# raufs/skDER

Hardware: NVIDIA B200
Metric: genome pairs/sec ANI+AF (higher is better)
Workload: dtype u64/int32 + f64

## Files before the change

### skder_b200/build.py

```python
import os
import subprocess
import sys

HERE = os.path.dirname(os.path.abspath(__file__))
CSRC = os.path.join(HERE, "csrc")
LIBDIR = os.path.join(HERE, "_lib")
LIB = os.path.join(LIBDIR, "libskani_b200.so")
SOURCES = ["skb_api.cu", "fasta_pack.cpp"]
HEADERS = ["skb_common.cuh", "skb_sketch.cuh", "skb_index.cuh", "skb_probe.cuh", "skb_ani.cuh", "../../include/skani_b200.h"]


def _stale():
    if not os.path.exists(LIB):
        return True
    t = os.path.getmtime(LIB)
    return any(os.path.getmtime(os.path.join(CSRC, f)) > t for f in SOURCES + HEADERS)


def build(force=False, verbose=False):
    if not force and not _stale():
        return LIB
    os.makedirs(LIBDIR, exist_ok=True)
    nvcc = os.environ.get("NVCC", "/usr/local/cuda/bin/nvcc")
    cmd = [
        nvcc, "-O3", "-std=c++17",
        "-gencode", "arch=compute_100a,code=sm_100a",
        "-lineinfo", "-Xcompiler", "-fPIC", "-shared",
        "-o", LIB,
    ] + [os.path.join(CSRC, s) for s in SOURCES] + ["-lz"]
    if verbose:
        cmd.insert(1, "-Xptxas=-v")
        print(" ".join(cmd), file=sys.stderr)
    subprocess.check_call(cmd)
    return LIB


if __name__ == "__main__":
    print(build(force="--force" in sys.argv, verbose=True))
```

### skder_b200/csrc/skb_api.cu

```cuda
#include <cuda_runtime.h>

#include <algorithm>
#include <cmath>
#include <cstdio>
#include <cstdlib>
#include <cstring>
#include <ctime>
#include <cub/cub.cuh>
#include <map>
#include <string>
#include <thread>
#include <vector>

#include "skb_ani.cuh"
#include "skb_common.cuh"
#include "skb_index.cuh"
#include "skb_sketch.cuh"

using namespace skb;

namespace {

thread_local std::string g_create_error;

struct CudaFail {
    std::string msg;
};

#define CK(call)                                                                                          \
    do {                                                                                                  \
        cudaError_t e__ = (call);                                                                         \
        if (e__ != cudaSuccess)                                                                           \
            throw CudaFail{std::string(#call) + ": " + cudaGetErrorString(e__) + " (" + __FILE__ + ":" + \
                           std::to_string(__LINE__) + ")"};                                               \
    } while (0)

template <typename T>
struct DevBuf {
    T *p = nullptr;
    size_t cap = 0;
    ~DevBuf() { release(); }
    void release() {
        if (p) cudaFree(p);
        p = nullptr;
        cap = 0;
    }
    void reserve(size_t n, size_t keep, cudaStream_t st) {
        if (n <= cap) return;
        size_t ncap = std::max(n, cap + cap / 2);
        T *q = nullptr;
        CK(cudaMalloc(&q, ncap * sizeof(T)));
        if (p && keep) CK(cudaMemcpyAsync(q, p, keep * sizeof(T), cudaMemcpyDeviceToDevice, st));
        if (p) {
            CK(cudaStreamSynchronize(st));
            cudaFree(p);
        }
        p = q;
        cap = ncap;
    }
    void upload(const std::vector<T> &h, size_t from, cudaStream_t st) {
        reserve(std::max<size_t>(h.size(), 1), from, st);
        if (h.size() > from)
            CK(cudaMemcpyAsync(p + from, h.data() + from, (h.size() - from) * sizeof(T), cudaMemcpyHostToDevice, st));
    }
};

template <typename T>
struct PoolRef {
    DevBuf<unsigned char> &b;
// ... 41 lines not shown
        int32_t n() const { return (int32_t)total_len.size(); }
        template <typename L>
        void append(uint64_t n_seeds, uint64_t len, const L *ctg_lens, size_t n_ctg) {
            seed_off.push_back(seed_off.back() + n_seeds);
            total_len.push_back(len);
            for (size_t k = 0; k < n_ctg; k++) ctg_len.push_back((uint32_t)ctg_lens[k]);
            ctg_off.push_back((uint32_t)ctg_len.size());
        }
        void truncate(int32_t n, uint64_t mkeys) {
            seed_off.resize(n + 1);
            total_len.resize(n);
            ctg_off.resize(n + 1);
            ctg_len.resize(ctg_off.back());
            n_mkeys = mkeys;
        }
        void clear() { *this = SketchDb(); }
    } db;
    struct HostIndex {
        int32_t n_indexed = 0;
        int32_t n_inv_genomes = 0;
        uint64_t n_inv = 0;
        uint64_t n_mkeys_indexed = 0;
        std::vector<uint64_t> tab_off{0}, marker_off{0};
        std::vector<uint32_t> chunk_off{0};
        std::vector<uint32_t> tab_buckets;
        std::vector<uint32_t> ctg_pstart, chunk_start, chunk_len;

        void truncate(const SketchDb &db) {
            const int32_t n = db.n();
            if (n_indexed <= n) return;
            n_indexed = n;
            tab_off.resize(n + 1);
            tab_buckets.resize(n);
            ctg_pstart.resize(db.ctg_len.size());
            chunk_off.resize(n + 1);
            chunk_start.resize(chunk_off.back());
            chunk_len.resize(chunk_off.back());
            marker_off.resize(n + 1);
            n_mkeys_indexed = std::min(n_mkeys_indexed, db.n_mkeys);
        }
        void clear() { *this = HostIndex(); }
    } ix;
    DevBuf<uint64_t> d_seeds, d_mkeys;
    bool indexed = false;
    int32_t own_first = 0, own_count = -1;
    int32_t kept_n = 0;
    uint64_t kept_seeds = 0;
    int kept_x2 = 0;
    int tab_x2 = 4;
    int tab_x2_forced = 0;
    int x2_decided = 0;
    uint64_t x2_decided_seeds = 0;
    DevBuf<uint64_t> d_seed_off, d_tab, d_tab_off, d_total_len, d_inv, d_markers, d_marker_off;
    DevBuf<uint32_t> d_tab_buckets;
    DevBuf<uint32_t> d_chunk_begin, d_chunk_start, d_chunk_len, d_chunk_off, d_ctg_pstart, d_ctg_len, d_ctg_off,
        d_marker_cnt;
    struct AddCall { int32_t n_before; uint64_t mkeys_before; };
    std::vector<AddCall> add_calls;
    DevBuf<unsigned char> d_tmp;
    std::map<std::string, DevBuf<unsigned char>> pool;
    DevBuf<int> d_counter;
    DevBuf<PairInfo> d_info;
    DevBuf<uint32_t> d_nch, d_task_off;

    int32_t n() const { return db.n(); }
    bool owns(int32_t g) const { return own_count < 0 || (g >= own_first && g < own_first + own_count); }
    std::pair<int32_t, int32_t> owned_in(int32_t g0, int32_t n) const {
        const int32_t o0 = std::clamp(own_count < 0 ? g0 : own_first, g0, n);
        return {o0, std::clamp(own_count < 0 ? n : own_first + own_count, o0, n)};
    }
    DbView view() const {
        DbView v;
        v.n_genomes = ix.n_indexed;
        v.seeds = d_seeds.p;
        v.g_seed_off = d_seed_off.p;
        v.tab = d_tab.p;
        v.g_tab_off = d_tab_off.p;
        v.g_tab_buckets = d_tab_buckets.p;
        v.chunk_begin = d_chunk_begin.p;
        v.chunk_start = d_chunk_start.p;
        v.chunk_len = d_chunk_len.p;
        v.g_chunk_off = d_chunk_off.p;
        v.ctg_pstart = d_ctg_pstart.p;
        v.ctg_len = d_ctg_len.p;
        v.g_ctg_off = d_ctg_off.p;
        v.g_total_len = d_total_len.p;
        v.markers = d_markers.p;
        v.g_marker_off = d_marker_off.p;
        v.inv_keys = d_inv.p;
        v.n_inv = (int64_t)ix.n_inv;
        return v;
    }
    AniParams ani_params() const {
        AniParams a;
        a.band_bp = prm.band_bp;
        a.max_gap = prm.max_gap;
        a.anchor_score = prm.anchor_score;
        a.min_anchors = prm.min_anchors;
        a.min_score = prm.min_score;
        a.max_mult = prm.max_mult;
        a.max_chunk_chains = prm.max_chunk_chains;
        a.ovl_num = prm.ovl_num;
        a.ovl_den = prm.ovl_den;
        a.span_ext = prm.span_ext;
        a.debias_a = prm.debias_a;
        a.debias_g = prm.debias_g;
        return a;
    }
};

namespace {

template <typename F>
int guarded(skb_ctx *ctx, F &&f) {
    if (!ctx) return SKB_EINVAL;
    try {
        CK(cudaSetDevice(ctx->device));
        return f();
    } catch (const CudaFail &e) {
        ctx->err = e.msg;
        return SKB_ECUDA;
    } catch (const std::bad_alloc &) {
        ctx->err = "host out of memory";
        return SKB_ENOMEM;
    } catch (const std::exception &e) {
        ctx->err = e.what();
        return SKB_EINVAL;
    }
// ... 100 lines not shown
    CK(cudaGetLastError());
    c->launches++;
    exclusive_scan_u32(c, d_cnt_s.p, d_off_s.p, n_warps + 1);
    exclusive_scan_u32(c, d_cnt_m.p, d_off_m.p, n_warps + 1);
    std::vector<uint32_t> h_off_s(nb + 1);
    uint32_t tot_m = 0;
    PoolRef<uint32_t> d_goff(c->pool["sketch_batch.d_goff"]);
    d_goff.reserve((size_t)nb + 1, 0, c->st);
    gather_strided_kernel<<<nblk((uint64_t)nb + 1, 256), 256, 0, c->st>>>(d_off_s.p, b.tile_off, SK_WARPS, nb + 1, d_goff.p);
    CK(cudaGetLastError());
    c->launches++;
    CK(cudaMemcpyAsync(h_off_s.data(), d_goff.p, ((size_t)nb + 1) * 4, cudaMemcpyDeviceToHost, c->st));
    CK(cudaMemcpyAsync(&tot_m, d_off_m.p + n_warps, 4, cudaMemcpyDeviceToHost, c->st));
    CK(cudaStreamSynchronize(c->st));
    const uint64_t cur_seeds = c->db.seed_off.back();
    const uint64_t tot_s = h_off_s[nb];
    c->d_seeds.reserve(cur_seeds + tot_s + 1, cur_seeds, c->st);
    c->d_mkeys.reserve(c->db.n_mkeys + tot_m + 1, c->db.n_mkeys, c->st);
    sketch_kernel<true><<<n_tiles, SK_THREADS, 0, c->st>>>(b, nullptr, nullptr, d_off_s.p, d_off_m.p,
                                                           c->d_seeds.p + cur_seeds, c->d_mkeys.p + c->db.n_mkeys,
                                                           d_masks.p);
    CK(cudaGetLastError());
    c->launches++;
    CK(cudaStreamSynchronize(c->st));
    for (int32_t i = 0; i < nb; i++) {
        const skb_packed *p = gen[g0 + i];
        c->db.append(h_off_s[i + 1] - h_off_s[i], (uint64_t)p->n_bases, p->contig_lens, (size_t)p->n_contigs);
    }
    c->db.n_mkeys += tot_m;
    c->indexed = false;
}

constexpr int EST_SORT_LAUNCHES = 4;

void run_ani(skb_ctx *c, const unsigned long long *d_pairs, int64_t n_pairs, PairOut *d_out) {
    c->anchor_ev_used = 0;
    if (n_pairs == 0) return;
    if (n_pairs >= (1ll << 31)) throw CudaFail{"too many surviving pairs in one call"};
    static const uint32_t fw_cap = [] {
        const char *e = std::getenv("SKB_FW_CAP");
        const int v = e ? atoi(e) : 1024;
        uint32_t w = 32;
        while ((int)w < v && w < 4096) w <<= 1;
        return w;
    }();
    const size_t fw_smem = (size_t)FW_WARPS * ((fw_bytes_per_warp(fw_cap) + 15) & ~(size_t)15);
    if (!c->ani_attr_set) {
        CK(cudaFuncSetAttribute(finalize_kernel<false, false>, cudaFuncAttributeMaxDynamicSharedMemorySize,
                                (int)(FIN_BYTES_PER_CAND * MAXP)));
        CK(cudaFuncSetAttribute(finalize_kernel<false, true>, cudaFuncAttributeMaxDynamicSharedMemorySize,
                                (int)(FIN_BYTES_PER_CAND * MAXP)));
        CK(cudaFuncSetAttribute(finalize_warp_kernel<false>, cudaFuncAttributeMaxDynamicSharedMemorySize, (int)fw_smem));
        CK(cudaFuncSetAttribute(finalize_warp_kernel<true>, cudaFuncAttributeMaxDynamicSharedMemorySize, (int)fw_smem));
        c->ani_attr_set = true;
    }
    const bool est = c->estimator != SKB_ANI_MEAN;
    const DbView view = c->view();
    const AniParams prm = c->ani_params();
    c->d_info.reserve((size_t)n_pairs, 0, c->st);
    c->d_nch.reserve((size_t)n_pairs + 1, 0, c->st);
    c->d_task_off.reserve((size_t)n_pairs + 1, 0, c->st);
    PoolRef<unsigned long long> d_key(c->pool["run_ani.key"]), d_key2(c->pool["run_ani.key2"]);
    PoolRef<uint32_t> d_idx(c->pool["run_ani.idx"]), d_perm(c->pool["run_ani.perm"]);
    PoolRef<PairInfo> d_info_s(c->pool["run_ani.info_sorted"]);
    d_key.reserve((size_t)n_pairs, 0, c->st);
    d_key2.reserve((size_t)n_pairs, 0, c->st);
    d_idx.reserve((size_t)n_pairs, 0, c->st);
    d_perm.reserve((size_t)n_pairs, 0, c->st);
    d_info_s.reserve((size_t)n_pairs, 0, c->st);
    pair_setup_kernel<<<nblk((uint64_t)n_pairs, 256), 256, 0, c->st>>>(view, d_pairs, n_pairs, c->d_info.p, d_key.p,
                                                                      d_idx.p);
    CK(cudaGetLastError());
    {
        size_t bytes = 0;
        CK(cub::DeviceRadixSort::SortPairs(nullptr, bytes, d_key.p, d_key2.p, d_idx.p, d_perm.p, (int64_t)n_pairs, 0, 64,
                                           c->st));
        c->d_tmp.reserve(bytes + 16, 0, c->st);
        CK(cub::DeviceRadixSort::SortPairs(c->d_tmp.p, bytes, d_key.p, d_key2.p, d_idx.p, d_perm.p, (int64_t)n_pairs, 0,
                                           64, c->st));
    }
    pair_gather_kernel<<<nblk((uint64_t)n_pairs, 256), 256, 0, c->st>>>(c->d_info.p, d_perm.p, n_pairs, d_info_s.p,
                                                                       c->d_nch.p);
    CK(cudaGetLastError());
    c->launches += 11;
    CK(cudaMemsetAsync(c->d_nch.p + n_pairs, 0, 4, c->st));
    exclusive_scan_u32(c, c->d_nch.p, c->d_task_off.p, (size_t)n_pairs + 1);
    std::vector<uint32_t> h_nch((size_t)n_pairs);
    CK(cudaMemcpyAsync(h_nch.data(), c->d_nch.p, (size_t)n_pairs * 4, cudaMemcpyDeviceToHost, c->st));
    CK(cudaStreamSynchronize(c->st));
    uint64_t total_tasks = 0;
    for (uint32_t v : h_nch) total_tasks += v;
    static const uint64_t batch_tasks = [] {
        const char *e = std::getenv("SKB_PAIR_BATCH_TASKS");
        return (uint64_t)(e ? std::max(1 << 16, atoi(e)) : (5 << 20));
    }();
    const uint64_t want_batches = std::max<uint64_t>(1, (total_tasks + batch_tasks / 2) / batch_tasks);
    const uint64_t max_tasks = std::min<uint64_t>(8ull << 20, (total_tasks + want_batches - 1) / want_batches + 4096);
    struct Batch { int64_t p0, p1; uint64_t base, tasks; };
    std::vector<Batch> batches;
    {
        int64_t p0 = 0;
        uint64_t base = 0;
        while (p0 < n_pairs) {
            uint64_t tasks = 0;
            int64_t p1 = p0;
            while (p1 < n_pairs && (p1 == p0 || tasks + h_nch[(size_t)p1] <= max_tasks)) tasks += h_nch[(size_t)p1++];
            if (tasks >= (1ull << 32)) throw CudaFail{"one pair has more than 2^32 query chunks"};
            batches.push_back({p0, p1, base, tasks});
            base += tasks;
            p0 = p1;
        }
    }
    uint64_t cap = 1;
    int64_t cap_pairs = 1;
    for (const Batch &bt : batches) {
        cap = std::max(cap, bt.tasks);
        cap_pairs = std::max(cap_pairs, bt.p1 - bt.p0);
    }
    PoolRef<uint64_t> b_anc(c->pool["ani.anc"]);
    PoolRef<uint32_t> b_res(c->pool["ani.res"]), b_next(c->pool["ani.next"]), b_fctl(c->pool["ani.fin_ctl"]),
        b_big_list(c->pool["ani.big_list"]), b_big_nc(c->pool["ani.big_nc"]), b_mid_list(c->pool["ani.mid_list"]);
    PoolRef<uint16_t> b_tn(c->pool["ani.tn"]);
    PoolRef<TaskDesc> b_desc(c->pool["ani.desc"]);
    PoolRef<Cand> b_cands(c->pool["ani.cands"]);
    PoolRef<PCand> b_pcands(c->pool["ani.pcands"]);
    PoolRef<uint32_t> b_task_pair(c->pool["ani.task_pair"]), b_cand_off(c->pool["ani.cand_off"]);
    PoolRef<uint8_t> b_ncand(c->pool["ani.ncand"]);
    PoolRef<uint32_t> b_slow(c->pool["ani.slow_list"]);
    b_anc.reserve(slab_entries(cap) + 2, 0, c->st);
    b_res.reserve(slab_entries(cap), 0, c->st);
    b_tn.reserve((size_t)cap, 0, c->st);
    b_desc.reserve((size_t)cap, 0, c->st);
    b_cands.reserve((size_t)cap * SLOTS, 0, c->st);
    b_pcands.reserve((size_t)cap * SLOTS, 0, c->st);
    b_task_pair.reserve((size_t)cap, 0, c->st);
    b_cand_off.reserve((size_t)cap + 1, 0, c->st);
    b_ncand.reserve((size_t)cap + 1, 0, c->st);
    b_slow.reserve((size_t)cap + 1, 0, c->st);
    b_next.reserve(1, 0, c->st);
    b_fctl.reserve(4, 0, c->st);
    b_mid_list.reserve((size_t)cap_pairs, 0, c->st);
    b_big_list.reserve((size_t)cap_pairs, 0, c->st);
    b_big_nc.reserve((size_t)cap_pairs, 0, c->st);
    PoolRef<uint8_t> e_acc(c->pool["est.acc"]);
    if (est) e_acc.reserve((size_t)cap * SLOTS, 0, c->st);
    bool wide_diag = std::getenv("SKB_WIDE_DIAG") != nullptr && atoi(std::getenv("SKB_WIDE_DIAG")) != 0;
    for (int32_t g = 0; g < c->ix.n_indexed && !wide_diag; g++) {
        const uint32_t k1 = c->db.ctg_off[(size_t)g + 1];
        if (k1 > c->db.ctg_off[(size_t)g] &&
            (uint64_t)c->ix.ctg_pstart[k1 - 1] + c->db.ctg_len[k1 - 1] >= (1ull << 30) - (1ull << 21))
            wide_diag = true;
    }
    static const bool trace = std::getenv("SKB_TRACE") != nullptr;
    struct Span { const char *name; size_t batch; cudaEvent_t e0, e1; };
    std::vector<Span> spans;
    cudaEvent_t ev_t0 = nullptr;
    auto mark = [&]() {
        cudaEvent_t e = nullptr;
        if (trace) {
            CK(cudaEventCreate(&e));
            CK(cudaEventRecord(e, c->st));
        }
        return e;
    };
    if (trace) ev_t0 = mark();
    for (size_t bi = 0; bi < batches.size(); bi++) {
        const Batch &bt = batches[bi];
        const int64_t np = bt.p1 - bt.p0;
        const uint32_t tasks = (uint32_t)bt.tasks, base = (uint32_t)bt.base;
        CK(cudaMemsetAsync(b_fctl.p, 0, 16, c->st));
        if (tasks) {
            CK(cudaMemsetAsync(b_ncand.p, 0, (size_t)tasks + 1, c->st));
            CK(cudaMemsetAsync(b_slow.p, 0, 4, c->st));
            CK(cudaMemsetAsync(b_next.p, 0, 4, c->st));
            task_setup_kernel<<<nblk(tasks, 256), 256, 0, c->st>>>(view, d_info_s.p + bt.p0, c->d_task_off.p + bt.p0, base, np,
                                                                   tasks, b_desc.p, b_task_pair.p);
            CK(cudaGetLastError());
            const unsigned g1 = std::min<unsigned>(nblk(tasks, (ANC_THREADS / 32) * ANC_GRAB), (unsigned)c->sm_count * 32u);
            if ((int)c->anchor_ev.size() < c->anchor_ev_used + 2) {
                cudaEvent_t e0, e1;
                CK(cudaEventCreate(&e0));
                CK(cudaEventCreate(&e1));
                c->anchor_ev.push_back(e0);
                c->anchor_ev.push_back(e1);
            }
            CK(cudaEventRecord(c->anchor_ev[c->anchor_ev_used], c->st));
            cudaEvent_t t0 = mark();
            if (wide_diag)
                anchor_kernel<false><<<g1, ANC_THREADS, 0, c->st>>>(view, prm, b_desc.p, tasks, b_anc.p, b_tn.p, b_next.p);
            else
                anchor_kernel<true><<<g1, ANC_THREADS, 0, c->st>>>(view, prm, b_desc.p, tasks, b_anc.p, b_tn.p, b_next.p);
            CK(cudaGetLastError());
            if (trace) spans.push_back({"anchor", bi, t0, mark()});
            CK(cudaEventRecord(c->anchor_ev[c->anchor_ev_used + 1], c->st));
            c->anchor_ev_used += 2;
            t0 = mark();
            if (wide_diag)
                chain_kernel<true><<<nblk(tasks, DP_THREADS), DP_THREADS, 0, c->st>>>(prm, tasks, b_anc.p, b_tn.p, b_res.p, b_desc.p,
                                                                                      b_cands.p, b_ncand.p, b_slow.p);
            else
                chain_kernel<false><<<nblk(tasks, DP_THREADS), DP_THREADS, 0, c->st>>>(prm, tasks, b_anc.p, b_tn.p, b_res.p, b_desc.p,
                                                                                       b_cands.p, b_ncand.p, b_slow.p);
            CK(cudaGetLastError());
            if (trace) spans.push_back({"chain", bi, t0, mark()});
            const unsigned g3 = std::min<unsigned>(nblk(tasks, END_THREADS / 32), (unsigned)c->sm_count * 4u);
            ends_kernel<<<g3, END_THREADS, 0, c->st>>>(prm, tasks, b_anc.p, b_res.p, b_tn.p, b_desc.p, b_slow.p, b_cands.p,
                                                       b_ncand.p);
            CK(cudaGetLastError());
            c->launches += 4;
        }
        cudaEvent_t tf = mark();
        if (tasks) {
            exclusive_scan_u8(c, b_ncand.p, b_cand_off.p, (size_t)tasks + 1);
            cand_pack_kernel<<<nblk(tasks, 256), 256, 0, c->st>>>(view, prm, d_info_s.p + bt.p0, tasks, b_task_pair.p, b_ncand.p,
                                                                  b_cand_off.p, b_cands.p, b_pcands.p);
            CK(cudaGetLastError());
            c->launches += 1;
        }
        (est ? finalize_warp_kernel<true> : finalize_warp_kernel<false>)<<<nblk((uint64_t)np, FW_WARPS), FW_WARPS * 32, fw_smem,
                                                                          c->st>>>(
            view, prm, d_info_s.p + bt.p0, c->d_task_off.p + bt.p0, base, np, b_pcands.p, b_cand_off.p, d_perm.p + bt.p0, d_out,
            fw_cap, b_fctl.p, b_mid_list.p, b_big_list.p, b_big_nc.p, e_acc.p);
        CK(cudaGetLastError());
        uint32_t fctl[4] = {0, 0, 0, 0};
        uint32_t n_cand = 0;
        CK(cudaMemcpyAsync(fctl, b_fctl.p, 16, cudaMemcpyDeviceToHost, c->st));
        if (est && tasks) CK(cudaMemcpyAsync(&n_cand, b_cand_off.p + tasks, 4, cudaMemcpyDeviceToHost, c->st));
        CK(cudaStreamSynchronize(c->st));
        c->launches += 1;
        if (fctl[2]) {
            uint32_t fcap = 32;
            while (fcap < fctl[0]) fcap <<= 1;
            (est ? finalize_kernel<false, true> : finalize_kernel<false, false>)<<<fctl[2], FIN_THREADS,
                                                                                  FIN_BYTES_PER_CAND * (size_t)fcap, c->st>>>(
                view, prm, d_info_s.p + bt.p0, c->d_task_off.p + bt.p0, base, np, b_pcands.p, b_cand_off.p,
                d_perm.p + bt.p0, d_out, fcap, b_mid_list.p, nullptr, nullptr, nullptr, e_acc.p);
            CK(cudaGetLastError());
            c->launches += 1;
        }
        if (fctl[1]) {
            const uint32_t nbig = fctl[1];
// ... 375 lines not shown
}


static int table_density(skb_ctx *c, uint64_t own_seeds) {
    if (c->tab_x2_forced) return c->tab_x2_forced;
    if (c->x2_decided && c->x2_decided_seeds == own_seeds) return c->x2_decided;
    size_t free_b = 0, total_b = 0;
    CK(cudaMemGetInfo(&free_b, &total_b));
    const double budget = std::min(0.35 * (double)total_b,
                                   (double)free_b + (double)c->d_tab.cap * 8.0 - 40.0 * (double)(1ull << 30));
    c->x2_decided = 1;
    for (int x2 : {4, 2})
        if (((double)own_seeds * x2 / 2 + (double)c->n()) * BUCKET * 8.0 <= budget) {
            c->x2_decided = x2;
            break;
        }
    c->x2_decided_seeds = own_seeds;
    return c->x2_decided;
}

static int build_seed_tables(skb_ctx *c, int32_t g0, bool reuse) {
    const int32_t n = c->n();
    std::vector<uint64_t> &tab_off = c->ix.tab_off;
    std::vector<uint32_t> &buckets = c->ix.tab_buckets;
    tab_off.resize(n + 1);
    buckets.resize(n);
    for (int32_t g = g0; g < n; g++) {
        const uint64_t ns = c->db.seed_off[g + 1] - c->db.seed_off[g];
        if (ns >= (1ull << 31)) return fail(c, SKB_ELIMIT, "genome has too many seeds");
        buckets[g] = c->owns(g) ? (uint32_t)std::max<uint64_t>(2, ns * (uint64_t)c->tab_x2 / 2 + 1) : 0u;
        tab_off[g + 1] = tab_off[g] + (uint64_t)buckets[g] * BUCKET;
    }
    c->d_seed_off.upload(c->db.seed_off, g0, c->st);
    c->d_tab_off.upload(tab_off, g0, c->st);
    c->d_tab_buckets.upload(buckets, g0, c->st);
    const uint64_t t0 = tab_off[g0], t1 = tab_off[n];
    c->d_tab.reserve(t1 + BUCKET, reuse ? t1 : t0, c->st);
    if (reuse) return SKB_OK;
    CK(cudaMemsetAsync(c->d_tab.p + t0, 0xFF, (t1 - t0) * 8, c->st));
    const auto [o0, o1] = c->owned_in(g0, n);
    const uint64_t s0 = c->db.seed_off[o0], s1 = c->db.seed_off[o1];
    if (s1 > s0) {
        tab_insert_kernel<<<nblk(s1 - s0, 256), 256, 0, c->st>>>(c->d_seeds.p, s1, c->d_seed_off.p, n, c->d_tab.p,
                                                               c->d_tab_off.p, c->d_tab_buckets.p, s0);
        CK(cudaGetLastError());
        rep_flag_kernel<<<nblk(s1 - s0, 256), 256, 0, c->st>>>(c->d_seeds.p, s1, c->d_seed_off.p, n, c->d_tab.p,
                                                             c->d_tab_off.p, c->d_tab_buckets.p, c->prm.max_mult, s0);
        CK(cudaGetLastError());
        c->launches += 2;
    }
    return SKB_OK;
}

static int build_chunk_tables(skb_ctx *c, int32_t g0) {
    const int32_t n = c->n();
    const uint32_t CL = (uint32_t)c->prm.chunk_len;
    const skb_ctx::SketchDb &db = c->db;
    skb_ctx::HostIndex &ix = c->ix;
    ix.chunk_off.resize(n + 1);
    for (int32_t g = g0; g < n; g++) {
        uint64_t cnt = 0;
        for (uint32_t k = db.ctg_off[g]; k < db.ctg_off[g + 1]; k++) cnt += (db.ctg_len[k] + CL - 1) / CL;
        if ((uint64_t)ix.chunk_off[g] + cnt >= (1ull << 32)) return fail(c, SKB_ELIMIT, "too many chunks");
        ix.chunk_off[g + 1] = ix.chunk_off[g] + (uint32_t)cnt;
    }
    ix.ctg_pstart.resize(db.ctg_len.size());
    ix.chunk_start.resize(ix.chunk_off[n]);
    ix.chunk_len.resize(ix.chunk_off[n]);
    auto fill = [&](int32_t ga, int32_t gb) {
        for (int32_t g = ga; g < gb; g++) {
            uint32_t off = 0, at = ix.chunk_off[g];
            for (uint32_t k = db.ctg_off[g]; k < db.ctg_off[g + 1]; k++) {
                ix.ctg_pstart[k] = off;
                const uint32_t len = db.ctg_len[k];
                for (uint32_t st = 0; st < len; st += CL, at++) {
                    ix.chunk_start[at] = off + st;
                    ix.chunk_len[at] = std::min<uint32_t>(CL, len - st);
                }
                off += len + CONTIG_PAD;
            }
        }
    };
    const int64_t m = n - g0;
    const int n_thr = m >= 1024 ? 4 : 1;
    if (n_thr == 1)
        fill(g0, n);
    else {
        std::vector<std::thread> pool;
        for (int t = 0; t < n_thr; t++)
            pool.emplace_back(fill, g0 + (int32_t)(m * t / n_thr), g0 + (int32_t)(m * (t + 1) / n_thr));
        for (auto &th : pool) th.join();
    }
    const size_t k0 = db.ctg_off[g0], ch0 = ix.chunk_off[g0];
    c->d_total_len.upload(db.total_len, g0, c->st);
    c->d_ctg_off.upload(db.ctg_off, g0, c->st);
    c->d_ctg_len.upload(db.ctg_len, k0, c->st);
    c->d_ctg_pstart.upload(ix.ctg_pstart, k0, c->st);
    c->d_chunk_off.upload(ix.chunk_off, g0, c->st);
    c->d_chunk_start.upload(ix.chunk_start, ch0, c->st);
    c->d_chunk_len.upload(ix.chunk_len, ch0, c->st);
    const uint32_t e0 = (uint32_t)ch0 + (uint32_t)g0, e1 = ix.chunk_off[n] + (uint32_t)n;
    c->d_chunk_begin.reserve(e1, e0, c->st);
    chunk_begin_kernel<<<nblk(e1 - e0, 256), 256, 0, c->st>>>(c->d_seeds.p, c->d_seed_off.p, c->d_chunk_off.p, n,
                                                             c->d_chunk_start.p, c->d_chunk_begin.p, e1, e0);
    CK(cudaGetLastError());
    c->launches++;
    return SKB_OK;
}

static void marker_offsets(skb_ctx *c, int32_t g0) {
    const int32_t n = c->n();
    std::vector<uint32_t> cnt((size_t)(n - g0));
    CK(cudaMemcpyAsync(cnt.data(), c->d_marker_cnt.p + g0, cnt.size() * 4, cudaMemcpyDeviceToHost, c->st));
    CK(cudaStreamSynchronize(c->st));
    std::vector<uint64_t> &off = c->ix.marker_off;
    off.resize(n + 1);
    for (int32_t g = g0; g < n; g++) off[g + 1] = off[g] + cnt[(size_t)(g - g0)];
    c->d_marker_off.upload(off, g0, c->st);
    CK(cudaStreamSynchronize(c->st));
}

int skb_index(skb_ctx *ctx) {
    return guarded(ctx, [&]() -> int {
        skb_ctx *c = ctx;
        static const bool trace = std::getenv("SKB_TRACE") != nullptr;
        double t_last = 0;
        auto lap = [&](const char *what) {
            if (!trace) return;
            cudaStreamSynchronize(c->st);
            timespec ts;
            clock_gettime(CLOCK_MONOTONIC, &ts);
            const double now = ts.tv_sec * 1e3 + ts.tv_nsec * 1e-6;
            if (what) fprintf(stderr, "[skb trace] index %-14s %7.2f ms\n", what, now - t_last);
            t_last = now;
        };
        lap(nullptr);
        const int32_t n = c->n();
        if (n == 0) return fail(c, SKB_ESTATE, "no genomes added");
        const auto [o0, o1] = c->owned_in(0, n);
        const uint64_t own_seeds = c->db.seed_off[o1] - c->db.seed_off[o0];
        const bool reuse = c->kept_n > 0 && c->kept_n == o1 - o0 && c->kept_seeds == own_seeds;
        c->tab_x2 = reuse ? c->kept_x2 : table_density(c, own_seeds);
        int rc = build_seed_tables(c, 0, reuse);
        if (rc != SKB_OK) return rc;
        c->kept_n = 0;
        lap("seed tables");
        if ((rc = build_chunk_tables(c, 0)) != SKB_OK) return rc;
        lap("chunk tables");
        c->d_marker_cnt.reserve((size_t)n, 0, c->st);
        CK(cudaMemsetAsync(c->d_marker_cnt.p, 0, (size_t)n * 4, c->st));
        c->ix.n_inv = 0;
        const uint64_t nk = c->db.n_mkeys;
        if (nk) {
            if (nk >= (1ull << 32)) return fail(c, SKB_ELIMIT, "too many marker keys");
            PoolRef<uint64_t> d_sorted(c->pool["skb_index.d_sorted"]);
            PoolRef<uint32_t> d_flag(c->pool["skb_index.d_flag"]), d_pos(c->pool["skb_index.d_pos"]);
            d_sorted.reserve(nk, 0, c->st);
            d_flag.reserve(nk + 1, 0, c->st);
            d_pos.reserve(nk + 1, 0, c->st);
            sort_keys_u64(c, c->d_mkeys.p, d_sorted.p, nk, 64, GID_BITS);
            unique_flag_kernel<<<nblk(nk, 256), 256, 0, c->st>>>(d_sorted.p, nk, d_flag.p);
            CK(cudaGetLastError());
            CK(cudaMemsetAsync(d_flag.p + nk, 0, 4, c->st));
            exclusive_scan_u32(c, d_flag.p, d_pos.p, nk + 1);
            uint32_t nu = 0;
            CK(cudaMemcpyAsync(&nu, d_pos.p + nk, 4, cudaMemcpyDeviceToHost, c->st));
            CK(cudaStreamSynchronize(c->st));
            c->ix.n_inv = nu;
            c->d_inv.reserve(nu + 1, 0, c->st);
            unique_scatter_kernel<<<nblk(nk, 256), 256, 0, c->st>>>(d_sorted.p, nk, d_flag.p, d_pos.p, c->d_inv.p,
                                                                  c->d_marker_cnt.p);
            CK(cudaGetLastError());
            c->launches += 3;
            lap("inverted index");
            c->d_markers.reserve(nu + 1, 0, c->st);
            swap_key_kernel<<<nblk(nu, 256), 256, 0, c->st>>>(c->d_inv.p, nu, d_sorted.p);
            CK(cudaGetLastError());
            sort_keys_u64(c, d_sorted.p, c->d_markers.p, nu, 64, 2 * K_MARKER);
            strip_gid_kernel<<<nblk(nu, 256), 256, 0, c->st>>>(c->d_markers.p, nu);
            CK(cudaGetLastError());
            c->launches += 3;
        }
        marker_offsets(c, 0);
        lap("marker lists");
        c->ix.n_indexed = n;
        c->ix.n_inv_genomes = n;
        c->ix.n_mkeys_indexed = nk;
        c->indexed = true;
        return SKB_OK;
    });
}

int skb_index_seed_tables(skb_ctx *ctx) {
    return guarded(ctx, [&]() -> int {
        skb_ctx *c = ctx;
        const int32_t n = c->n();
        if (n == 0) return fail(c, SKB_ESTATE, "no genomes added");
        const auto [o0, o1] = c->owned_in(0, n);
        const uint64_t own_seeds = c->db.seed_off[o1] - c->db.seed_off[o0];
        c->tab_x2 = table_density(c, own_seeds);
        const int rc = build_seed_tables(c, 0, false);
        if (rc != SKB_OK) return rc;
        CK(cudaStreamSynchronize(c->st));
        c->kept_n = o1 - o0;
        c->kept_seeds = own_seeds;
        c->kept_x2 = c->tab_x2;
        c->indexed = false;
        return SKB_OK;
    });
}

int skb_index_append(skb_ctx *ctx) {
    return guarded(ctx, [&]() -> int {
        skb_ctx *c = ctx;
        const int32_t n = c->n(), n0 = c->ix.n_indexed;
        if (!c->indexed && n0 == 0) return fail(c, SKB_ESTATE, "call skb_index on the database first");
        if (n == n0) {
            c->indexed = true;
            return SKB_OK;
        }
        int rc = build_seed_tables(c, n0, false);
        if (rc != SKB_OK) return rc;
        if ((rc = build_chunk_tables(c, n0)) != SKB_OK) return rc;
        const uint64_t nk = c->db.n_mkeys - c->ix.n_mkeys_indexed;
        c->d_marker_cnt.reserve((size_t)n, (size_t)n0, c->st);
        CK(cudaMemsetAsync(c->d_marker_cnt.p + n0, 0, (size_t)(n - n0) * 4, c->st));
        if (nk) {
            PoolRef<uint64_t> d_a(c->pool["skb_index_append.a"]), d_b(c->pool["skb_index_append.b"]);
            PoolRef<uint32_t> d_flag(c->pool["skb_index_append.flag"]), d_pos(c->pool["skb_index_append.pos"]);
            d_a.reserve(nk, 0, c->st);
            d_b.reserve(nk, 0, c->st);
            d_flag.reserve(nk + 1, 0, c->st);
            d_pos.reserve(nk + 1, 0, c->st);
            swap_key_kernel<<<nblk(nk, 256), 256, 0, c->st>>>(c->d_mkeys.p + c->ix.n_mkeys_indexed, nk, d_a.p);
            CK(cudaGetLastError());
            sort_keys_u64(c, d_a.p, d_b.p, nk);
            unique_flag_kernel<<<nblk(nk, 256), 256, 0, c->st>>>(d_b.p, nk, d_flag.p);
            CK(cudaGetLastError());
            CK(cudaMemsetAsync(d_flag.p + nk, 0, 4, c->st));
            exclusive_scan_u32(c, d_flag.p, d_pos.p, nk + 1);
            uint32_t nu = 0;
            CK(cudaMemcpyAsync(&nu, d_pos.p + nk, 4, cudaMemcpyDeviceToHost, c->st));
            CK(cudaStreamSynchronize(c->st));
            const uint64_t m0 = c->ix.marker_off[n0];
            c->d_markers.reserve(m0 + nu + 1, m0, c->st);
            unique_scatter_swapped_kernel<<<nblk(nk, 256), 256, 0, c->st>>>(d_b.p, nk, d_flag.p, d_pos.p, c->d_markers.p + m0,
                                                                           c->d_marker_cnt.p);
            CK(cudaGetLastError());
            c->launches += 3;
        }
        marker_offsets(c, n0);
        c->ix.n_mkeys_indexed = c->db.n_mkeys;
        c->ix.n_indexed = n;
        c->indexed = true;
        return SKB_OK;
    });
}

int skb_pop_last_add(skb_ctx *ctx) {
    return guarded(ctx, [&]() -> int {
        skb_ctx *c = ctx;
        if (c->add_calls.empty()) return fail(c, SKB_ESTATE, "nothing to pop");
        const skb_ctx::AddCall a = c->add_calls.back();
        if (a.n_before < c->ix.n_inv_genomes) return fail(c, SKB_ESTATE, "cannot pop genomes that are part of the inverted index");
        CK(cudaStreamSynchronize(c->st));
        c->add_calls.pop_back();
        c->db.truncate(a.n_before, a.mkeys_before);
        c->ix.truncate(c->db);
        c->indexed = c->ix.n_indexed == a.n_before && a.n_before > 0;
        return SKB_OK;
    });
}

int skb_sketch_sizes(skb_ctx *ctx, int32_t g, int64_t *n_seeds, int64_t *n_markers, int32_t *n_chunks,
                     int64_t *total_len) {
// ... 639 lines not shown
```

### skder_b200/csrc/skb_common.cuh

```cuda
#pragma once
#include <cuda_runtime.h>
#include <stdint.h>

#include "../../include/skani_b200.h"

namespace skb {

constexpr int K_SEED = 15;
constexpr int K_MARKER = 21;
constexpr uint64_t C_SEED = 125;
constexpr uint64_t C_MARKER = 1000;
constexpr uint64_t THR_SEED = 0xFFFFFFFFFFFFFFFFull / C_SEED;
constexpr uint64_t THR_MARKER = 0xFFFFFFFFFFFFFFFFull / C_MARKER;
constexpr uint64_t MASK_MARKER = (~0ull) >> (64 - 2 * K_MARKER);
constexpr uint64_t MASK_SEED = (~0ull) >> (64 - 2 * K_SEED);
constexpr uint32_t CONTIG_PAD = 4096;

__host__ __device__ inline uint32_t seed_kmer(uint64_t s) { return (uint32_t)(s >> 34); }
__host__ __device__ inline uint32_t seed_pos(uint64_t s) { return (uint32_t)((s >> 2) & 0xffffffffu); }
__host__ __device__ inline int seed_rep(uint64_t s) { return (int)((s >> 1) & 1); }
__host__ __device__ inline int seed_strand(uint64_t s) { return (int)(s & 1); }

constexpr int GID_BITS = 22;
constexpr uint64_t GID_MASK = (1ull << GID_BITS) - 1;

constexpr uint64_t TAB_EMPTY = 0xFFFFFFFFFFFFFFFFull;

__host__ __device__ inline uint64_t mm_hash64(uint64_t key) {
    key = ~(key * 0x200001ull);
    key = key ^ (key >> 24);
    key = key * 265ull;
    key = key ^ (key >> 14);
    key = key * 21ull;
    key = key ^ (key >> 28);
    key = key * 0x80000001ull;
    return key;
}

__host__ __device__ inline uint32_t row_owner(uint32_t a, uint32_t P) {
    const uint32_t m = a % (2 * P);
    return m < P ? m : 2 * P - 1 - m;
}
__host__ __device__ inline uint32_t row_local(uint32_t a, uint32_t P) { return 2 * (a / (2 * P)) + (a % (2 * P) >= P ? 1u : 0u); }
__host__ __device__ inline uint32_t row_global(uint32_t rl, uint32_t part, uint32_t P) {
    return (rl >> 1) * 2 * P + ((rl & 1) ? 2 * P - 1 - part : part);
}
__host__ __device__ inline uint32_t rows_owned(uint32_t n, uint32_t part, uint32_t P) {
    const uint32_t rem = n % (2 * P);
    return 2 * (n / (2 * P)) + (rem > part ? 1u : 0u) + (rem > 2 * P - 1 - part ? 1u : 0u);
}

constexpr uint32_t BUCKET = 4;

constexpr int SLAB = 256;
__host__ __device__ inline size_t slab_base(uint32_t t) { return (size_t)t * SLAB; }
__host__ __device__ inline uint32_t slab_off(uint32_t i) { return i; }
__host__ __device__ inline size_t slab_entries(uint64_t tasks) { return (size_t)tasks * SLAB; }

struct DbView {
    int32_t n_genomes;
    const uint64_t *seeds;
    const uint64_t *g_seed_off;
    const uint64_t *tab;
    const uint64_t *g_tab_off;
    const uint32_t *g_tab_buckets;
    const uint32_t *chunk_begin;
    const uint32_t *chunk_start;
    const uint32_t *chunk_len;
    const uint32_t *g_chunk_off;
    const uint32_t *ctg_pstart;
    const uint32_t *ctg_len;
    const uint32_t *g_ctg_off;
    const uint64_t *g_total_len;
    const uint64_t *markers;
    const uint64_t *g_marker_off;
    const uint64_t *inv_keys;
    int64_t n_inv;
};

struct PairOut {
    double ani, ani_raw, af_q, af_r;
    int64_t n_anchors, n_seeds, span_q, span_r;
    int32_t n_chains, swapped;
};

}
```

### skder_b200/csrc/skb_index.cuh

```cuda
#pragma once
#include "skb_common.cuh"
#include "skb_probe.cuh"

namespace skb {

__global__ void chunk_begin_kernel(const uint64_t *__restrict__ seeds, const uint64_t *__restrict__ g_seed_off,
                                   const uint32_t *__restrict__ g_chunk_off, int n_genomes,
                                   const uint32_t *__restrict__ chunk_start, uint32_t *__restrict__ chunk_begin,
                                   uint32_t total_entries , uint32_t first) {
    uint32_t t = first + blockIdx.x * blockDim.x + threadIdx.x;
    if (t >= total_entries) return;
    int lo = 0, hi = n_genomes - 1;
    while (lo < hi) {
        int mid = (lo + hi + 1) >> 1;
        if (g_chunk_off[mid] + (uint32_t)mid <= t)
            lo = mid;
        else
            hi = mid - 1;
    }
    const int g = lo;
    const uint32_t local = t - (g_chunk_off[g] + g);
    const uint32_t nch = g_chunk_off[g + 1] - g_chunk_off[g];
    const uint64_t *S = seeds + g_seed_off[g];
    const uint32_t ns = (uint32_t)(g_seed_off[g + 1] - g_seed_off[g]);
    if (local == nch) {
        chunk_begin[t] = ns;
        return;
    }
    const uint32_t start = chunk_start[g_chunk_off[g] + local];
    uint32_t l = 0, h = ns;
    while (l < h) {
        uint32_t mid = (l + h) >> 1;
        if (seed_pos(S[mid]) < start)
            l = mid + 1;
        else
            h = mid;
    }
    chunk_begin[t] = l;
}

__global__ void unique_flag_kernel(const uint64_t *__restrict__ keys, uint64_t n, uint32_t *__restrict__ flag) {
    uint64_t i = (uint64_t)blockIdx.x * blockDim.x + threadIdx.x;
    if (i >= n) return;
    flag[i] = (i == 0 || keys[i] != keys[i - 1]) ? 1u : 0u;
}
__global__ void unique_scatter_kernel(const uint64_t *__restrict__ keys, uint64_t n,
                                      const uint32_t *__restrict__ flag, const uint32_t *__restrict__ pos,
                                      uint64_t *__restrict__ out, uint32_t *__restrict__ g_marker_cnt) {
    uint64_t i = (uint64_t)blockIdx.x * blockDim.x + threadIdx.x;
    if (i >= n || !flag[i]) return;
    out[pos[i]] = keys[i];
    atomicAdd(&g_marker_cnt[keys[i] & GID_MASK], 1u);
}
__global__ void swap_key_kernel(const uint64_t *__restrict__ inv, uint64_t n, uint64_t *__restrict__ out) {
    uint64_t i = (uint64_t)blockIdx.x * blockDim.x + threadIdx.x;
    if (i >= n) return;
    const uint64_t k = inv[i];
    out[i] = ((k & GID_MASK) << (2 * K_MARKER)) | (k >> GID_BITS);
}
__global__ void unique_scatter_swapped_kernel(const uint64_t *__restrict__ keys, uint64_t n,
                                              const uint32_t *__restrict__ flag, const uint32_t *__restrict__ pos,
                                              uint64_t *__restrict__ out, uint32_t *__restrict__ g_marker_cnt) {
    uint64_t i = (uint64_t)blockIdx.x * blockDim.x + threadIdx.x;
    if (i >= n || !flag[i]) return;
    out[pos[i]] = keys[i] & MASK_MARKER;
    atomicAdd(&g_marker_cnt[keys[i] >> (2 * K_MARKER)], 1u);
}
__global__ void strip_gid_kernel(uint64_t *keys, uint64_t n) {
    uint64_t i = (uint64_t)blockIdx.x * blockDim.x + threadIdx.x;
    if (i < n) keys[i] &= MASK_MARKER;
}

__global__ void screen_runs_kernel(const uint64_t *__restrict__ inv, uint64_t n, uint32_t *cnt, uint32_t n_genomes,
                                   int part, int n_parts, uint32_t row0, uint32_t n_rows) {
    uint64_t i = (uint64_t)blockIdx.x * blockDim.x + threadIdx.x;
    if (i >= n) return;
    const uint64_t k = inv[i];
    const uint32_t gi = (uint32_t)(k & GID_MASK);
    if ((int)row_owner(gi, (uint32_t)n_parts) != part) return;
    const uint32_t rl = row_local(gi, (uint32_t)n_parts) - row0;
    if (rl >= n_rows) return;
    const uint64_t m = k >> GID_BITS;
    uint32_t *row = cnt + (size_t)rl * n_genomes;
    for (uint64_t j = i + 1; j < n; j++) {
        const uint64_t kj = inv[j];
        if ((kj >> GID_BITS) != m) break;
        atomicAdd(row + (uint32_t)(kj & GID_MASK), 1u);
    }
}

__global__ void screen_compact_kernel(const uint32_t *__restrict__ cnt, uint32_t n_genomes, uint32_t n_rows_local,
// ... 148 lines not shown
```

Measured before the change: 174.1 million.

## Replace hash-probe anchor finding with sorted-merge join per genome pair

Adds a per-genome sorted copy of seeds, keyed by k-mer, with original ordinals, built by a segmented sort at index time. A new join kernel processes one genome pair per block. It streams reference seeds in shared-memory tiles, binary-searches query keys against each tile, and records hits into a shared-memory window indexed by query seed ordinal. It then emits anchors per chunk with warp ballots and prefix sums. This replaces the hash-table probe anchor kernel in the common case. The cost is extra index memory and build time, and it falls back when diagonals are wide or genomes exceed 2^27 seeds.

Measured after the change: 133.6 million (median of 6 runs). 0.767x the previous value.

```diff
diff --git a/skder_b200/build.py b/skder_b200/build.py
--- a/skder_b200/build.py
+++ b/skder_b200/build.py
@@ -7,7 +7,7 @@
 LIBDIR = os.path.join(HERE, "_lib")
 LIB = os.path.join(LIBDIR, "libskani_b200.so")
 SOURCES = ["skb_api.cu", "fasta_pack.cpp"]
-HEADERS = ["skb_common.cuh", "skb_sketch.cuh", "skb_index.cuh", "skb_probe.cuh", "skb_ani.cuh", "../../include/skani_b200.h"]
+HEADERS = ["skb_common.cuh", "skb_sketch.cuh", "skb_index.cuh", "skb_probe.cuh", "skb_ani.cuh", "skb_join.cuh", "../../include/skani_b200.h"]
 
 
 def _stale():
diff --git a/skder_b200/csrc/skb_api.cu b/skder_b200/csrc/skb_api.cu
--- a/skder_b200/csrc/skb_api.cu
+++ b/skder_b200/csrc/skb_api.cu
@@ -15,6 +15,7 @@
 #include "skb_ani.cuh"
 #include "skb_common.cuh"
 #include "skb_index.cuh"
+#include "skb_join.cuh"
 #include "skb_sketch.cuh"
 
 using namespace skb;
@@ -162,6 +163,8 @@
     int x2_decided = 0;
     uint64_t x2_decided_seeds = 0;
     DevBuf<uint64_t> d_seed_off, d_tab, d_tab_off, d_total_len, d_inv, d_markers, d_marker_off;
+    DevBuf<uint64_t> d_sseeds;
+    DevBuf<uint32_t> d_sord;
     DevBuf<uint32_t> d_tab_buckets;
     DevBuf<uint32_t> d_chunk_begin, d_chunk_start, d_chunk_len, d_chunk_off, d_ctg_pstart, d_ctg_len, d_ctg_off,
         d_marker_cnt;
@@ -184,6 +187,8 @@
         v.n_genomes = ix.n_indexed;
         v.seeds = d_seeds.p;
         v.g_seed_off = d_seed_off.p;
+        v.sseeds = d_sseeds.p;
+        v.sord = d_sord.p;
         v.tab = d_tab.p;
         v.g_tab_off = d_tab_off.p;
         v.g_tab_buckets = d_tab_buckets.p;
@@ -390,6 +395,7 @@
                                 (int)(FIN_BYTES_PER_CAND * MAXP)));
         CK(cudaFuncSetAttribute(finalize_warp_kernel<false>, cudaFuncAttributeMaxDynamicSharedMemorySize, (int)fw_smem));
         CK(cudaFuncSetAttribute(finalize_warp_kernel<true>, cudaFuncAttributeMaxDynamicSharedMemorySize, (int)fw_smem));
+        CK(cudaFuncSetAttribute(join_anchor_kernel, cudaFuncAttributeMaxDynamicSharedMemorySize, (int)JN_SMEM));
         c->ani_attr_set = true;
     }
     const bool est = c->estimator != SKB_ANI_MEAN;
@@ -489,6 +495,9 @@
             (uint64_t)c->ix.ctg_pstart[k1 - 1] + c->db.ctg_len[k1 - 1] >= (1ull << 30) - (1ull << 21))
             wide_diag = true;
     }
+    bool join = !wide_diag && !(std::getenv("SKB_ANCHOR_PROBE") != nullptr && atoi(std::getenv("SKB_ANCHOR_PROBE")) != 0);
+    for (int32_t g = 0; g < c->ix.n_indexed && join; g++)
+        if (c->db.seed_off[(size_t)g + 1] - c->db.seed_off[(size_t)g] >= (1ull << JN_IDX_BITS)) join = false;
     static const bool trace = std::getenv("SKB_TRACE") != nullptr;
     struct Span { const char *name; size_t batch; cudaEvent_t e0, e1; };
     std::vector<Span> spans;
@@ -524,7 +533,10 @@
             }
             CK(cudaEventRecord(c->anchor_ev[c->anchor_ev_used], c->st));
             cudaEvent_t t0 = mark();
-            if (wide_diag)
+            if (join)
+                join_anchor_kernel<<<(unsigned)np, JN_THREADS, JN_SMEM, c->st>>>(view, prm, d_info_s.p + bt.p0,
+                                                                             c->d_task_off.p + bt.p0, base, b_anc.p, b_tn.p);
+            else if (wide_diag)
                 anchor_kernel<false><<<g1, ANC_THREADS, 0, c->st>>>(view, prm, b_desc.p, tasks, b_anc.p, b_tn.p, b_next.p);
             else
                 anchor_kernel<true><<<g1, ANC_THREADS, 0, c->st>>>(view, prm, b_desc.p, tasks, b_anc.p, b_tn.p, b_next.p);
@@ -1006,6 +1018,36 @@
     return SKB_OK;
 }
 
+static void build_sorted_seeds(skb_ctx *c, int32_t g0) {
+    const int32_t n = c->n();
+    const std::vector<uint64_t> &off = c->db.seed_off;
+    c->d_sseeds.reserve(off[n] + 1, off[g0], c->st);
+    c->d_sord.reserve(off[n] + 1, off[g0], c->st);
+    PoolRef<uint32_t> d_ord(c->pool["sorted_seeds.ord"]);
+    PoolRef<int64_t> d_seg(c->pool["sorted_seeds.seg"]);
+    for (int32_t ga = g0; ga < n;) {
+        int32_t gb = ga + 1;
+        while (gb < n && off[gb + 1] - off[ga] <= (1ull << 28)) gb++;
+        const uint64_t s0 = off[ga], m = off[gb] - s0;
+        if (m) {
+            std::vector<int64_t> seg((size_t)(gb - ga) + 1);
+            for (int32_t g = ga; g <= gb; g++) seg[(size_t)(g - ga)] = (int64_t)(off[g] - s0);
+            d_seg.upload(seg, c->st);
+            d_ord.reserve(m, 0, c->st);
+            seed_ordinal_kernel<<<nblk(m, 256), 256, 0, c->st>>>(c->d_seed_off.p, n, s0, s0 + m, d_ord.p);
+            CK(cudaGetLastError());
+            size_t bytes = 0;
+            CK(cub::DeviceSegmentedSort::SortPairs(nullptr, bytes, c->d_seeds.p + s0, c->d_sseeds.p + s0, d_ord.p,
+                                                   c->d_sord.p + s0, (int)m, gb - ga, d_seg.p, d_seg.p + 1, c->st));
+            c->d_tmp.reserve(bytes + 16, 0, c->st);
+            CK(cub::DeviceSegmentedSort::SortPairs(c->d_tmp.p, bytes, c->d_seeds.p + s0, c->d_sseeds.p + s0, d_ord.p,
+                                                   c->d_sord.p + s0, (int)m, gb - ga, d_seg.p, d_seg.p + 1, c->st));
+            c->launches += 1 + EST_SORT_LAUNCHES;
+        }
+        ga = gb;
+    }
+}
+
 static int build_chunk_tables(skb_ctx *c, int32_t g0) {
     const int32_t n = c->n();
     const uint32_t CL = (uint32_t)c->prm.chunk_len;
@@ -1099,6 +1141,8 @@
         if (rc != SKB_OK) return rc;
         c->kept_n = 0;
         lap("seed tables");
+        build_sorted_seeds(c, 0);
+        lap("sorted seeds");
         if ((rc = build_chunk_tables(c, 0)) != SKB_OK) return rc;
         lap("chunk tables");
         c->d_marker_cnt.reserve((size_t)n, 0, c->st);
@@ -1175,6 +1219,7 @@
         }
         int rc = build_seed_tables(c, n0, false);
         if (rc != SKB_OK) return rc;
+        build_sorted_seeds(c, n0);
         if ((rc = build_chunk_tables(c, n0)) != SKB_OK) return rc;
         const uint64_t nk = c->db.n_mkeys - c->ix.n_mkeys_indexed;
         c->d_marker_cnt.reserve((size_t)n, (size_t)n0, c->st);
diff --git a/skder_b200/csrc/skb_common.cuh b/skder_b200/csrc/skb_common.cuh
--- a/skder_b200/csrc/skb_common.cuh
+++ b/skder_b200/csrc/skb_common.cuh
@@ -61,6 +61,8 @@
     int32_t n_genomes;
     const uint64_t *seeds;
     const uint64_t *g_seed_off;
+    const uint64_t *sseeds;
+    const uint32_t *sord;
     const uint64_t *tab;
     const uint64_t *g_tab_off;
     const uint32_t *g_tab_buckets;
diff --git a/skder_b200/csrc/skb_index.cuh b/skder_b200/csrc/skb_index.cuh
--- a/skder_b200/csrc/skb_index.cuh
+++ b/skder_b200/csrc/skb_index.cuh
@@ -37,6 +37,13 @@
             h = mid;
     }
     chunk_begin[t] = l;
+}
+
+__global__ void seed_ordinal_kernel(const uint64_t *__restrict__ g_seed_off, int n_genomes, uint64_t first,
+                                    uint64_t end, uint32_t *__restrict__ out) {
+    const uint64_t i = first + (uint64_t)blockIdx.x * blockDim.x + threadIdx.x;
+    const int g = genome_of_warp(g_seed_off, n_genomes, i < end ? i : end - 1);
+    if (i < end) out[i - first] = (uint32_t)(i - g_seed_off[g]);
 }
 
 __global__ void unique_flag_kernel(const uint64_t *__restrict__ keys, uint64_t n, uint32_t *__restrict__ flag) {
diff --git a/skder_b200/csrc/skb_join.cuh b/skder_b200/csrc/skb_join.cuh
--- /dev/null
+++ b/skder_b200/csrc/skb_join.cuh
@@ -0,0 +1,211 @@
+#pragma once
+#include "skb_ani.cuh"
+
+namespace skb {
+
+constexpr int JN_THREADS = 1024;
+constexpr int JN_Q = 4;
+constexpr int JN_WAVE = JN_THREADS * JN_Q;
+constexpr int JN_RT = 4096;
+constexpr int JN_W = 45056;
+constexpr int JN_CH = 512;
+constexpr size_t JN_SMEM = (size_t)(JN_W + 2 * JN_RT + 2 * JN_CH + 1) * 4;
+constexpr int JN_IDX_BITS = 27;
+
+constexpr uint32_t HIT_NONE = 0xffffffffu;
+
+__device__ __forceinline__ uint32_t hit_of_rec(uint32_t lo) { return ((lo >> 1) & ~1u) | (lo & 1u); }
+
+__global__ void __launch_bounds__(JN_THREADS, 1)
+join_anchor_kernel(DbView db, AniParams prm, const PairInfo *__restrict__ info, const uint32_t *__restrict__ task_off,
+                   uint32_t base, uint64_t *__restrict__ anc_all, uint16_t *__restrict__ task_n) {
+    extern __shared__ uint32_t jsm[];
+    uint32_t *const hit = jsm;
+    uint32_t *const rk = jsm + JN_W;
+    uint32_t *const rv = rk + JN_RT;
+    uint32_t *const s_cb = rv + JN_RT;
+    uint32_t *const s_cs = s_cb + JN_CH + 1;
+    const int tid = threadIdx.x, lane = tid & 31, warp = tid >> 5;
+    const PairInfo pi = info[blockIdx.x];
+    const uint32_t t0 = task_off[blockIdx.x] - base;
+    const uint64_t qoff = db.g_seed_off[pi.q], roff = db.g_seed_off[pi.r];
+    const uint32_t nq = (uint32_t)(db.g_seed_off[pi.q + 1] - qoff), nr = (uint32_t)(db.g_seed_off[pi.r + 1] - roff);
+    const uint2 *__restrict__ qpos = reinterpret_cast<const uint2 *>(db.seeds + qoff);
+    const uint2 *__restrict__ qsrt = reinterpret_cast<const uint2 *>(db.sseeds + qoff);
+    const uint32_t *__restrict__ qord = db.sord + qoff;
+    const uint2 *__restrict__ rsrt = reinterpret_cast<const uint2 *>(db.sseeds + roff);
+    const uint32_t choff = db.g_chunk_off[pi.q];
+    const uint32_t *__restrict__ cbeg = db.chunk_begin + choff + pi.q;
+    const uint32_t nch = pi.nch;
+    const uint32_t cap = (uint32_t)prm.max_mult + 1;
+
+    for (uint32_t c0 = 0; c0 < nch;) {
+        const uint32_t w0 = cbeg[c0];
+        uint32_t lo = c0 + 1, hi = min(nch, c0 + (uint32_t)JN_CH);
+        while (lo < hi) {
+            const uint32_t mid = (lo + hi + 1) >> 1;
+            if (cbeg[mid] - w0 <= (uint32_t)JN_W)
+                lo = mid;
+            else
+                hi = mid - 1;
+        }
+        const uint32_t c1 = lo, w1 = cbeg[c1];
+        __syncthreads();
+        for (uint32_t k = tid; k < w1 - w0; k += JN_THREADS) hit[k] = HIT_NONE;
+        for (uint32_t k = tid; k <= c1 - c0; k += JN_THREADS) {
+            s_cb[k] = cbeg[c0 + k];
+            if (k < c1 - c0) s_cs[k] = db.chunk_start[choff + c0 + k];
+        }
+
+        uint32_t a = 0;
+        uint32_t key[JN_Q], ord[JN_Q], keyn[JN_Q], ordn[JN_Q];
+        bool pend[JN_Q];
+#pragma unroll
+        for (int u = 0; u < JN_Q; u++) {
+            const uint32_t i = u * JN_THREADS + tid, i2 = i + JN_WAVE;
+            key[u] = i < nq ? qsrt[i].y : HIT_NONE;
+            ord[u] = i < nq ? qord[i] : 0u;
+            pend[u] = i < nq;
+            keyn[u] = i2 < nq ? qsrt[i2].y : HIT_NONE;
+            ordn[u] = i2 < nq ? qord[i2] : 0u;
+        }
+        uint2 rn[JN_RT / JN_THREADS];
+#pragma unroll
+        for (int u = 0; u < JN_RT / JN_THREADS; u++) {
+            const uint32_t j = u * JN_THREADS + tid;
+            rn[u] = j < nr ? rsrt[j] : make_uint2(0u, HIT_NONE);
+        }
+        for (uint32_t j0 = 0; j0 < nr && a < nq; j0 += JN_RT) {
+            const uint32_t nt = min((uint32_t)JN_RT, nr - j0);
+            __syncthreads();
+#pragma unroll
+            for (int u = 0; u < JN_RT / JN_THREADS; u++) {
+                const uint32_t k = u * JN_THREADS + tid;
+                rk[k] = rn[u].y;
+                rv[k] = hit_of_rec(rn[u].x);
+            }
+            __syncthreads();
+#pragma unroll
+            for (int u = 0; u < JN_RT / JN_THREADS; u++) {
+                const uint32_t j = j0 + JN_RT + u * JN_THREADS + tid;
+                rn[u] = j < nr ? rsrt[j] : make_uint2(0u, HIT_NONE);
+            }
+            const uint32_t kmax = rk[nt - 1];
+            for (;;) {
+                bool go[JN_Q], any = false;
+#pragma unroll
+                for (int u = 0; u < JN_Q; u++) {
+                    go[u] = pend[u] && key[u] <= kmax;
+                    any |= go[u];
+                }
+                if (__any_sync(0xffffffffu, any)) {
+                    uint32_t l[JN_Q];
+#pragma unroll
+                    for (int u = 0; u < JN_Q; u++) l[u] = 0;
+#pragma unroll
+                    for (uint32_t st = JN_RT / 2; st >= 1; st >>= 1)
+#pragma unroll
+                        for (int u = 0; u < JN_Q; u++)
+                            if (rk[l[u] + st - 1] < key[u]) l[u] += st;
+#pragma unroll
+                    for (int u = 0; u < JN_Q; u++) {
+                        if (!go[u]) continue;
+                        pend[u] = false;
+                        if (ord[u] - w0 >= w1 - w0) continue;
+                        uint32_t w = HIT_NONE;
+                        if (rk[l[u]] == key[u]) {
+                            uint32_t c = 1;
+                            for (; c < cap; c++) {
+                                const uint32_t jj = l[u] + c;
+                                const uint32_t kk = jj < nt ? rk[jj] : (j0 + jj < nr ? rsrt[j0 + jj].y : HIT_NONE);
+                                if (kk != key[u]) break;
+                            }
+                            w = c == 1 ? rv[l[u]] : (1u << 31) | (c << JN_IDX_BITS) | (j0 + l[u]);
+                        }
+                        hit[ord[u] - w0] = w;
+                    }
+                }
+                const bool left = pend[0] || pend[1] || pend[2] || pend[3];
+                if (__syncthreads_or(left)) break;
+                a += JN_WAVE;
+                if (a >= nq) break;
+#pragma unroll
+                for (int u = 0; u < JN_Q; u++) {
+                    const uint32_t i = a + u * JN_THREADS + tid, i2 = i + JN_WAVE;
+                    key[u] = keyn[u];
+                    ord[u] = ordn[u];
+                    pend[u] = i < nq;
+                    keyn[u] = i2 < nq ? qsrt[i2].y : HIT_NONE;
+                    ordn[u] = i2 < nq ? qord[i2] : 0u;
+                }
+            }
+        }
+        __syncthreads();
+
+        constexpr int JN_EB = 8;
+        const uint32_t *__restrict__ qlo = reinterpret_cast<const uint32_t *>(qpos);
+        for (uint32_t ch = c0 + warp; ch < c1; ch += JN_THREADS / 32) {
+            const uint32_t sb = s_cb[ch - c0], ns = s_cb[ch - c0 + 1] - sb;
+            int n = 0;
+            if (ns > 0) {
+                const uint32_t cstart = s_cs[ch - c0];
+                const uint32_t *hc = hit + (sb - w0);
+                uint64_t *anc = anc_all + slab_base(t0 + ch);
+                uint32_t mult = (uint32_t)prm.max_mult;
+                for (;;) {
+                    int nb = 0;
+                    for (uint32_t g0 = 0; g0 < ns; g0 += 32 * JN_EB) {
+                        uint32_t xs[JN_EB];
+#pragma unroll
+                        for (int k = 0; k < JN_EB; k++) {
+                            const uint32_t s = g0 + 32 * k + lane;
+                            xs[k] = s < ns ? qlo[2 * (size_t)(sb + s)] : 2u;
+                        }
+#pragma unroll
+                        for (int k = 0; k < JN_EB; k++) {
+                            if (g0 + 32 * k >= ns) break;
+                            const uint32_t sx = xs[k], s = g0 + 32 * k + lane;
+                            const uint32_t w = (sx & 2u) ? HIT_NONE : hc[s];
+                            uint32_t c = w == HIT_NONE ? 0u : (w >> 31) ? (w >> JN_IDX_BITS) & 15u : 1u;
+                            if (c > mult) c = 0;
+                            const uint32_t lo = (((sx >> 2) - cstart) << 17) | s;
+                            if (!__any_sync(0xffffffffu, c > 1)) {
+                                const unsigned has = __ballot_sync(0xffffffffu, c != 0);
+                                if (c) {
+                                    const int dst = nb + __popc(has & ((1u << lane) - 1u));
+                                    if (dst < MAXA)
+                                        __stcg(anc + slab_off((uint32_t)dst), ((uint64_t)(w >> 1) << 32) | lo | (((w ^ sx) & 1u) << 16));
+                                }
+                                nb += __popc(has);
+                                continue;
+                            }
+                            int pre = (int)c;
+#pragma unroll
+                            for (int d = 1; d < 32; d <<= 1) {
+                                const int u = __shfl_up_sync(0xffffffffu, pre, d);
+                                if (lane >= d) pre += u;
+                            }
+                            const int tot = __shfl_sync(0xffffffffu, pre, 31);
+                            pre -= (int)c;
+                            for (uint32_t x = 0; x < c; x++) {
+                                const uint32_t v = c == 1 ? w : hit_of_rec(rsrt[(w & ((1u << JN_IDX_BITS) - 1u)) + x].x);
+                                const int dst = nb + pre + (int)x;
+                                if (dst < MAXA)
+                                    __stcg(anc + slab_off((uint32_t)dst), ((uint64_t)(v >> 1) << 32) | lo | (((v ^ sx) & 1u) << 16));
+                            }
+                            nb += tot;
+                        }
+                    }
+                    n = nb;
+                    if (n <= MAXA || mult == 1) break;
+                    mult >>= 1;
+                }
+                if (n > MAXA || n < prm.min_anchors) n = 0;
+            }
+            if (lane == 0) task_n[t0 + ch] = (uint16_t)n;
+        }
+        c0 = c1;
+    }
+}
+
+}
```
